# gddickinson/neural_enhanced_super_resolution

Measured on AMD Instinct MI355X. Metric: output megapixels/sec, RealESRGAN_x2plus x2 upscale, higher is better.
Workload: dtype f32 (operands as f16 hi+lo pairs, 3 f16 MFMAs per product, f32 accumulate); 1 GPU; c2: 512x512->1024x1024 RealESRGAN_x2plus fp32 single tile; frames_in_flight_per_gpu=1, world_size=1, partition=independent frames, no data-path collective

## Files before the change

neural_enhanced_super_resolution_amd/csrc/rdb_f16x2.hip:

```cpp
#include <type_traits>

#include "f16x2_common.h"
#include "nesr_kernels.h"
#include "rdb_f16x2_schedule.h"

namespace nesr {

namespace {

#if defined(NESR_RDB_PAR) || defined(NESR_RDB_EPI_STEPS) || defined(NESR_RDB_DMAPRIO) || defined(NESR_RDB_YPRIO) || NESR_RDB_LAG == 0
#error "NESR_RDB_PAR, NESR_RDB_EPI_STEPS, NESR_RDB_DMAPRIO, NESR_RDB_YPRIO and NESR_RDB_LAG=0 were removed; the last commit that had them is 19ed2fc (tools/build_variant.sh 19ed2fc out.so -D... still builds it)"
#endif

#ifndef NESR_RDB_ABL
#define NESR_RDB_ABL 0
#endif
namespace abl {
constexpr bool no_poll = NESR_RDB_ABL & 1;
constexpr bool plain_loads = NESR_RDB_ABL & 2;
constexpr bool plain_stores = NESR_RDB_ABL & 4;
constexpr bool no_mfma = NESR_RDB_ABL & 8;
constexpr bool no_epilogue = NESR_RDB_ABL & 16;
constexpr bool no_in_dma = NESR_RDB_ABL & 32;
constexpr bool no_w_dma = NESR_RDB_ABL & 64;
constexpr bool no_barrier = NESR_RDB_ABL & 512;
constexpr bool no_dma = no_in_dma || no_w_dma;
}

#if NESR_RDB_ABL & 256
__device__ unsigned long long g_rdb_stamps[2][64][8];
__device__ unsigned long long g_rdb_taps[2][8][8];
__device__ unsigned long long g_rdb_arrive[12][8][2];
#define RARRIVE(w, step, ev) do { if (blockIdx.x == 77 && lane == 0 && (step) >= 20 && (step) < 28) { unsigned long long t_ = __builtin_amdgcn_s_memtime(); asm volatile("s_waitcnt lgkmcnt(0)" ::: "memory"); g_rdb_arrive[w][(step) - 20][ev] = t_; } } while (0)
#define RSTAMP(role, step, ev) do { if (blockIdx.x == 77 && lane == 0) { unsigned long long t_ = __builtin_amdgcn_s_memtime(); asm volatile("s_waitcnt lgkmcnt(0)" ::: "memory"); g_rdb_stamps[role][step][ev] = t_; } } while (0)
#define RMSTEP_INIT() int mstep = 0
#define RSTAMP_M(ev) do { if (wave == 1) RSTAMP(0, mstep, ev); } while (0)
#define RARRIVE_M(d, ev) RARRIVE(wave, mstep + (d), ev)
#define RMSTEP_NEXT() ++mstep
#define RKEEP(x, y) asm volatile("" :: "v"(x), "v"(y))
#define RTAPS_INIT() unsigned long long tt_[6]
#define RTAP(i, fence) do { tt_[i] = __builtin_amdgcn_s_memtime(); if (fence) __builtin_amdgcn_sched_barrier(0); } while (0)
#define RTAPS_WRITE() do { if (blockIdx.x == 77 && (wave == 1 || wave == 5) && lane == 0 && mstep >= 20 && mstep < 28) { \
    _Pragma("unroll") for (int i_ = 0; i_ < 6; ++i_) g_rdb_taps[wave == 5][mstep - 20][i_] = tt_[i_]; } } while (0)
#define RCLOCKS(step) do { if (((step) == 0 || (step) == RDB_STEPS - 1) && wave == 0 && blockIdx.x == 77 && lane == 0) { \
    const unsigned long long r_ = __builtin_amdgcn_s_memrealtime(), t_ = __builtin_amdgcn_s_memtime(); asm volatile("s_waitcnt lgkmcnt(0)" ::: "memory"); \
    g_rdb_stamps[1][(step) == 0 ? 62 : 63][0] = r_; g_rdb_stamps[1][(step) == 0 ? 62 : 63][1] = t_; } } while (0)
#define RSTAMP_RETIRED() do { asm volatile("s_waitcnt vmcnt(0)" ::: "memory"); if (wave == 1) RSTAMP(0, 61, 1); } while (0)
#else
#define RSTAMP(role, step, ev) do { } while (0)
#define RARRIVE(w, step, ev) do { } while (0)
#define RMSTEP_INIT() do { } while (0)
#define RSTAMP_M(ev) do { } while (0)
#define RARRIVE_M(d, ev) do { } while (0)
#define RMSTEP_NEXT() do { } while (0)
#define RKEEP(x, y) do { } while (0)
#define RTAPS_INIT() do { } while (0)
#define RTAP(i, fence) do { } while (0)
#define RTAPS_WRITE() do { } while (0)
#define RCLOCKS(step) do { } while (0)
#define RSTAMP_RETIRED() do { } while (0)
#endif

struct RdbArgs {
    const void* cur;
    long long chunk_bytes;
    void* out;
    const void* res2;
    float s1, s2;
    const void* w[5];
    const float* bias[5];
    int n, h, w_;
    unsigned* progress;
    unsigned epoch;
    unsigned* abort_flag;
    unsigned* status;
    unsigned long long timeout_ticks;
};

__device__ __forceinline__ void glds16_s_sc1(const char* sbase, unsigned voff, unsigned lds_dst) {
    unsigned keep;
    asm volatile(
        "s_mov_b32 %0, m0\n\t"
        "s_mov_b32 m0, %3\n\t"
        "s_nop 0\n\t"
        "global_load_lds_dwordx4 %1, %2 sc1\n\t"
        "s_mov_b32 m0, %0"
        : "=&s"(keep)
        : "v"(voff), "s"(sbase), "s"(lds_dst)
        : "memory");
}
__device__ __forceinline__ void store16_wt_s(const char* sbase, unsigned voff, uint4 v) {
    asm volatile("global_store_dwordx4 %0, %1, %2 sc1\n\ts_nop 1" ::"v"(voff), "v"(__builtin_bit_cast(f32x4, v)), "s"(sbase) : "memory");
}
__device__ __forceinline__ f32x4 load16_s(const char* sbase, unsigned voff) {
    return *(const __attribute__((address_space(1))) f32x4*)(sbase + voff);
}

__device__ __forceinline__ void wait_vmcnt_le(int k) {
    switch (k) {
        case 0: asm volatile("s_waitcnt vmcnt(0)" ::: "memory"); break;
        case 1: asm volatile("s_waitcnt vmcnt(1)" ::: "memory"); break;
        case 2: asm volatile("s_waitcnt vmcnt(2)" ::: "memory"); break;
        case 3: asm volatile("s_waitcnt vmcnt(3)" ::: "memory"); break;
        case 4: asm volatile("s_waitcnt vmcnt(4)" ::: "memory"); break;
        case 5: asm volatile("s_waitcnt vmcnt(5)" ::: "memory"); break;
        case 6: asm volatile("s_waitcnt vmcnt(6)" ::: "memory"); break;
        case 7: asm volatile("s_waitcnt vmcnt(7)" ::: "memory"); break;
        case 8: asm volatile("s_waitcnt vmcnt(8)" ::: "memory"); break;
        case 9: asm volatile("s_waitcnt vmcnt(9)" ::: "memory"); break;
        case 10: asm volatile("s_waitcnt vmcnt(10)" ::: "memory"); break;
        case 11: asm volatile("s_waitcnt vmcnt(11)" ::: "memory"); break;
        default: asm volatile("s_waitcnt vmcnt(12)" ::: "memory"); break;
    }
}

constexpr int RSLOTS = 4;
constexpr int W5_ROUNDS = 2 * W_ITEMS / (64 * 4);
static_assert(RSLOTS == 4 && RDB_STEP5 % RSLOTS == 0 && W5_ROUNDS * 64 * 4 == 2 * W_ITEMS, "conv5's slab pairs sit at ring positions 0,1 / 2,3 and fill whole DMA rounds");
constexpr int MW = 8;
constexpr int DW = 4;
constexpr int EPI_STEPS = 1;

__global__ __launch_bounds__(64 * (MW + DW), 3) void rdb_f16x2_kernel(RdbArgs a) {
    typedef Geo<4> G;
    constexpr int THREADS = G::THREADS, TH = G::TH;
    constexpr int IN_ITEMS = G::IN_ITEMS, IN_ROUNDS = G::IN_ROUNDS, IN_BYTES = G::IN_BYTES;
    constexpr int W_ROUNDS = (W_ITEMS + THREADS - 1) / THREADS;
    constexpr int WRING = RSLOTS * IN_BYTES;
    constexpr int BIAS = RSLOTS * (IN_BYTES + W_BYTES);
    static_assert(TH == MW, "one tile row per MFMA wave");
    extern __shared__ __attribute__((aligned(16))) char smem[];

    const int lane = threadIdx.x & 63;
    const int wave_all = __builtin_amdgcn_readfirstlane(threadIdx.x >> 6);
    const bool is_dma = wave_all >= MW;
    const bool is_cmp = !is_dma;
    const int wave = is_cmp ? wave_all : wave_all - MW;
    const int tid = wave * 64 + lane;

    const int tiles_x = (a.w_ + TW - 1) / TW;
    const int tiles_y = (a.h + TH - 1) / TH;
    const int total = tiles_x * tiles_y * a.n;
    const int tile = xcd_work_index(total);
    const int n = tile / (tiles_x * tiles_y);
    const int t2 = tile - n * tiles_x * tiles_y;
    const int ty = t2 / tiles_x, tx = t2 - ty * tiles_x;
    const int y0 = ty * TH, x0 = tx * TW;

    const int j16 = lane & 15, g4 = lane >> 4;
    auto advance = [](int& l, int& c) {
        const int nc = l == 4 ? 12 : 4 + 2 * l;
        if (++c == nc) { c = 0; ++l; }
    };

    if (is_dma) {
        if (wave == 0) RSTAMP(1, 61, 0);
        const unsigned lds_base = (unsigned)(size_t)(lds_char*)(smem);
        unsigned voff[IN_ROUNDS];
        unsigned okmask = 0;
        unsigned wavemask = 0;
        const int row0 = y0 > 0 ? y0 - 1 : 0;
        const char* in_img = static_cast<const char*>(a.cur) + ((size_t)n * a.h + row0) * a.w_ * 64;
        const unsigned* watch = nullptr;
        int kin = 0, kw = 0;
        if (lane < 9) {
            const int ny = ty + lane / 3 - 1, nx = tx + lane % 3 - 1;
            if (ny >= 0 && ny < tiles_y && nx >= 0 && nx < tiles_x) watch = a.progress + (n * tiles_y + ny) * tiles_x + nx;
        }
        {
            int p = tid >> 2;
            int py = p / PW, px = p - py * PW;
            const int sl = tid & 3;
#pragma unroll
            for (int i = 0; i < IN_ROUNDS; ++i) {
                const int k = tid + THREADS * i;
                const int sg = sl ^ (((px >> 2) & 1) << 1);
                const int Y = y0 - 1 + py, X = x0 - 1 + px;
                const bool has = k < IN_ITEMS;
                const bool ok = has && Y >= 0 && Y < a.h && X >= 0 && X < a.w_;
                voff[i] = ((unsigned)(Y - row0) * (unsigned)a.w_ + (unsigned)X) * 64u + sg * 16;
                okmask |= ok ? (1u << i) : 0u;
                if (__builtin_amdgcn_ballot_w64(ok) != 0ull) { wavemask |= 1u << i; ++kin; }
                if (has && !ok) {
#pragma unroll
                    for (int sl2 = 0; sl2 < RSLOTS; ++sl2) *reinterpret_cast<f32x4*>(smem + sl2 * IN_BYTES + k * 16) = f32x4{0.f, 0.f, 0.f, 0.f};
                }
                px += (THREADS / 4) % PW;
                py += (THREADS / 4) / PW;
                if (px >= PW) { px -= PW; py += 1; }
            }
#pragma unroll
            for (int j = 0; j < W_ROUNDS; ++j) kw += (wave * 64 + THREADS * j) < W_ITEMS ? 1 : 0;
        }
        unsigned seen = 0;
        bool gave_up = false;
        auto dma_w = [&](int l, int c, int wpos) {
            const char* wsrc = static_cast<const char*>(a.w[l]) + (size_t)c * W_BYTES;
#pragma unroll
            for (int j = 0; j < W_ROUNDS; ++j) {
                const int k = tid + THREADS * j;
                const unsigned dst = lds_base + WRING + wpos * W_BYTES + j * (THREADS * 16) + wave * 1024;
                if (k < W_ITEMS && !abl::no_w_dma) glds16_s(wsrc, (unsigned)k * 16u, __builtin_amdgcn_readfirstlane(dst));
            }
        };
        auto dma_w5 = [&](int c, int wpos) {
            const char* wsrc = static_cast<const char*>(a.w[4]) + (size_t)c * (2 * W_BYTES);
#pragma unroll
            for (int j = 0; j < W5_ROUNDS; ++j) {
                const unsigned dst = lds_base + WRING + wpos * W_BYTES + j * (THREADS * 16) + wave * 1024;
                if (!abl::no_w_dma) glds16_s(wsrc, (unsigned)(tid + THREADS * j) * 16u, __builtin_amdgcn_readfirstlane(dst));
            }
        };
        auto dma_in = [&](int c, int slot) {
            const unsigned need = c < 4 ? 0u : (unsigned)((c - 4) >> 1) + 1u;
            if (need > seen && !gave_up && !abl::no_poll) {
                const unsigned target = a.epoch + need;
                unsigned long long t0 = 0;
                for (unsigned it = 0;; ++it) {
                    const unsigned v = watch ? __hip_atomic_load(watch, __ATOMIC_RELAXED, __HIP_MEMORY_SCOPE_AGENT) : target;
                    if (__builtin_amdgcn_ballot_w64((int)(v - target) < 0) == 0ull) break;
                    if ((it & 63u) == 0u) {
                        const unsigned long long now = __builtin_amdgcn_s_memrealtime();
                        if (it == 0) t0 = now;
                        const unsigned ab = __hip_atomic_load(a.abort_flag, __ATOMIC_RELAXED, __HIP_MEMORY_SCOPE_AGENT);
                        if (ab != 0u || now - t0 > a.timeout_ticks) {
                            if (ab == 0u && lane == 0) __hip_atomic_store(a.abort_flag, 1u | ((unsigned)c << 8) | ((unsigned)tile << 16), __ATOMIC_RELAXED, __HIP_MEMORY_SCOPE_AGENT);
                            gave_up = true;
                            break;
                        }
                    }
                    __builtin_amdgcn_s_sleep(4);
                }
                seen = need;
            }
            const char* isrc = in_img + (long long)c * a.chunk_bytes;
#pragma unroll
            for (int i = 0; i < IN_ROUNDS; ++i) {
                const unsigned dst = lds_base + slot * IN_BYTES + i * (THREADS * 16) + wave * 1024;
                if (((wavemask >> i) & 1u) && !abl::no_in_dma) {
                    if ((okmask >> i) & 1u) {
                        if (abl::plain_loads) glds16_s(isrc, voff[i], __builtin_amdgcn_readfirstlane(dst));
                        else glds16_s_sc1(isrc, voff[i], __builtin_amdgcn_readfirstlane(dst));
                    }
                }
            }
        };
        int fl = 0, fc = 0;
#pragma unroll
        for (int i = 0; i < rdbs::IN_LEAD; ++i) {
            dma_w(0, i, i);
            dma_in(i, i);
            advance(fl, fc);
        }
        gave_up = *(const __attribute__((address_space(4))) unsigned*)a.abort_flag != 0u;
        asm volatile("s_waitcnt lgkmcnt(0)" ::: "memory");
        int fill = rdbs::IN_LEAD;
        int cl = 0, cc = 0;
        wait_vmcnt_le(abl::no_dma ? 0 : (rdbs::IN_LEAD - 1) * (kw + kin));
        int inflight = kw + kin;
        __builtin_amdgcn_s_barrier();
        asm volatile("" ::: "memory");
        for (int step = 0; step < RDB_STEPS; ++step) {
            if (wave == 0) RSTAMP(1, step, 0);
            RCLOCKS(step);
            wait_vmcnt_le(abl::no_dma ? 0 : inflight);
            if (wave == 0) RSTAMP(1, step, 1);
            RARRIVE(MW + wave, step, 0);
            if (!abl::no_barrier) __builtin_amdgcn_s_barrier();
            asm volatile("" ::: "memory");
            RARRIVE(MW + wave, step, 1);
            if (wave == 0) RSTAMP(1, step, 2);
            if (cc == EPI_STEPS && cl >= 1 && wave == 0 && lane == 0)
                __hip_atomic_store(a.progress + tile, a.epoch + (unsigned)cl, __ATOMIC_RELAXED, __HIP_MEMORY_SCOPE_AGENT);
            if (rdbs::w_pair(step)) {
                dma_w5(step + 1 - RDB_STEP5, ((step + 1) & 1) * 2);
            } else if (rdbs::w_slab(step)) {
                dma_w(fl, fc, fill);
            }
            for (int k = rdbs::in_end(step) - rdbs::in_end(step - 1); k > 0; --k) {
                dma_in(fc, fill);
                advance(fl, fc);
                fill = fill == RSLOTS - 1 ? 0 : fill + 1;
            }
            inflight = rdbs::tail_w(step) * kw + rdbs::tail_in(step) * kin;
            if (wave == 0) RSTAMP(1, step, 3);
            advance(cl, cc);
        }
        return;
    }

    const bool active = (y0 + wave) < a.h;
    if (wave == 1) RSTAMP(0, 61, 0);
    const bool fills_bias = wave < 6 && lane < 8;
    f32x4 bias_v = f32x4{0.f, 0.f, 0.f, 0.f};
    if (fills_bias) bias_v = *(const __attribute__((address_space(1))) f32x4*)(a.bias[wave < 4 ? wave : 4] + (wave == 5 ? 32 : 0) + 4 * lane);
    const int un = g4 >> 1, kh = g4 & 1;
    int b16[5][2], a16[5];
#pragma unroll
    for (int st_ = 0; st_ < 5; ++st_) {
#pragma unroll
        for (int nh = 0; nh < 2; ++nh) b16[st_][nh] = tap_pixel_offset(st_, wave, nh, j16, un, kh);
        a16[st_] = tap_weight_offset(st_, j16, un, kh);
    }
    int slot = 0;
    int wpos = 0;
    RMSTEP_INIT();
    typedef const __attribute__((address_space(3))) f32x4* lds_f32x4;
    const unsigned lds0 = (unsigned)(size_t)(lds_char*)(smem);
    unsigned bcur[5], aw012, aw3, aw4, aw4b;
#pragma unroll
    for (int t = 0; t < 5; ++t) bcur[t] = lds0 + (unsigned)b16[t][0];
    const unsigned xl4 = (unsigned)((un ^ 1) << 5);
    aw012 = lds0 + (unsigned)(WRING + a16[0]);
    aw3 = lds0 + (unsigned)(WRING + a16[3]);
    aw4 = lds0 + (unsigned)(WRING + a16[4]);
    aw4b = aw4 + (unsigned)un * 1024u;
    const int cbl = (g4 & 1) * 16 + (g4 >> 1) * 8;
    const int piece8 = ((g4 & 1) * 2 + (g4 >> 1)) * 8;
    const bool res2 = a.res2 != nullptr;
    f32x4 ep[2][2];
#pragma unroll
    for (int nh = 0; nh < 2; ++nh)
#pragma unroll
        for (int mt = 0; mt < 2; ++mt) ep[nh][mt] = f32x4{0.f, 0.f, 0.f, 0.f};
    int ep_l = -1;
    bool bad = false;
    auto unpack_res = [&](f32x4 rx, f32x4 rx1, f32x4& q0, f32x4& q1) {
        uint4 cx = __builtin_bit_cast(uint4, rx), cx1 = __builtin_bit_cast(uint4, rx1);
        regroup_pairs(cx, cx1);
        const f16x8 h = __builtin_bit_cast(f16x8, cx), lo = __builtin_bit_cast(f16x8, cx1);
#pragma unroll
        for (int i = 0; i < 4; ++i) {
            q0[i] = fmaf((float)lo[i], LO_INV, (float)h[i]);
            q1[i] = fmaf((float)lo[4 + i], LO_INV, (float)h[4 + i]);
        }
    };
    const long long row_bytes = (((long long)n * a.h + (y0 + wave)) * a.w_) * 64;
    unsigned lane_off[2];
    bool lane_ok[2];
#pragma unroll
    for (int nh = 0; nh < 2; ++nh) {
        const int X = x0 + 16 * nh + j16;
        lane_ok[nh] = X < a.w_;
        lane_off[nh] = (unsigned)(lane_ok[nh] ? X : 0) * 64u + (unsigned)piece8 * 2u;
    }
    auto uni = [](const char* p) -> const char* {
        const unsigned long long v = (unsigned long long)p;
        const unsigned lo = __builtin_amdgcn_readfirstlane((unsigned)v), hi = __builtin_amdgcn_readfirstlane((unsigned)(v >> 32));
        return (const char*)(((unsigned long long)hi << 32) | lo);
    };
    auto epi_half = [&](int l, const f32x4& e0, const f32x4& e1, int nh) {
        RSTAMP_M(3);
        const bool valid = lane_ok[nh];
        const unsigned voff = lane_off[nh];
        const char* bsrc = smem + BIAS + (l * 32 + cbl) * 4;
        f32x4 v0, v1;
        cout_exchange(e0, e1, v0, v1);
        v0 += *reinterpret_cast<const f32x4*>(bsrc);
        v1 += *reinterpret_cast<const f32x4*>(bsrc + 16);
        const int dchunk = 4 + 2 * l;
#pragma unroll
        for (int i = 0; i < 4; ++i) { v0[i] = fmaxf(v0[i], v0[i] * 0.2f); v1[i] = fmaxf(v1[i], v1[i] * 0.2f); }
        RKEEP(v0, v1);
        RSTAMP_M(4);
        uint4 cx, cx1;
        bool bad_here = false;
        split_regroup(v0, v1, cx, cx1, bad_here);
        bad |= bad_here && valid;
        RKEEP(__builtin_bit_cast(f32x4, cx), __builtin_bit_cast(f32x4, cx1));
        RSTAMP_M(5);
        if (valid) {
            const char* d0 = uni(static_cast<const char*>(a.cur) + (long long)dchunk * a.chunk_bytes + row_bytes);
            if (!abl::plain_stores) {
                store16_wt_s(d0, voff, cx);
                store16_wt_s(d0 + a.chunk_bytes, voff, cx1);
            } else {
                *reinterpret_cast<uint4*>(const_cast<char*>(d0) + voff) = cx;
                *reinterpret_cast<uint4*>(const_cast<char*>(d0) + a.chunk_bytes + voff) = cx1;
            }
        }
        RSTAMP_M(6);
    };
    auto epi_pending = [&]() {
        if (abl::no_epilogue) return;
        epi_half(ep_l, ep[0][0], ep[0][1], 0);
        epi_half(ep_l, ep[1][0], ep[1][1], 1);
    };
    f32x4 R1[4][2], R2[4][2];
    auto issue_res = [&](const void* base, int g, f32x4 (&R)[4][2]) {
        const char* r = uni(static_cast<const char*>(base) + (long long)(2 * g) * a.chunk_bytes + row_bytes);
#pragma unroll
        for (int nh = 0; nh < 2; ++nh) {
            R[2 * g + nh][0] = load16_s(r, lane_off[nh]);
            R[2 * g + nh][1] = load16_s(r + a.chunk_bytes, lane_off[nh]);
        }
    };
    f32x4 acc16[2][2][2][2];
    f32x4 Af[2][2][2];
    f32x4 Bf[2][2][2];
    auto load_a = [&](int s_, int buf, unsigned off) {
#pragma unroll
        for (int mt = 0; mt < 2; ++mt) {
            if (s_ < 4) {
                const unsigned ad = s_ < 3 ? aw012 + s_ * 2048 : aw3;
                Af[buf][mt][0] = *((lds_f32x4)(size_t)(ad + off + mt * 256));
                Af[buf][mt][1] = *((lds_f32x4)(size_t)(ad + off + mt * 256 + 1024));
            } else {
                f32x4 hi = *((lds_f32x4)(size_t)(aw4 + off + mt * 256));
                Af[buf][mt][1] = *((lds_f32x4)(size_t)(aw4b + off + mt * 256));
                if (un) hi = f32x4{0.f, 0.f, 0.f, 0.f};
                Af[buf][mt][0] = hi;
            }
        }
    };
    auto move_a = [&](unsigned d) {
        aw012 += d;
        aw3 += d;
        aw4 += d;
        aw4b += d;
    };
    auto load_b = [&](int sl, int s_, int buf) {
        const unsigned dB = sl == RSLOTS - 1 ? (unsigned)(-(RSLOTS - 1) * IN_BYTES) : (unsigned)IN_BYTES;
        const unsigned xl = bcur[s_] ^ (s_ == 4 ? xl4 : 32u);
#pragma unroll
        for (int nh = 0; nh < 2; ++nh) {
            Bf[buf][nh][0] = *((lds_f32x4)(size_t)(bcur[s_] + nh * 1024));
            Bf[buf][nh][1] = *((lds_f32x4)(size_t)(xl + nh * 1024));
        }
        bcur[s_] += dB;
    };
    auto mfma_tap = [&](int s_, int g, int abuf, int bbuf) {
#pragma unroll
        for (int mt = 0; mt < 2; ++mt) {
            const f16x8 a0 = __builtin_bit_cast(f16x8, Af[abuf][mt][0]), a1 = __builtin_bit_cast(f16x8, Af[abuf][mt][1]);
#pragma unroll
            for (int nh = 0; nh < 2; ++nh) {
                const f16x8 x0_ = __builtin_bit_cast(f16x8, Bf[bbuf][nh][0]), x1_ = __builtin_bit_cast(f16x8, Bf[bbuf][nh][1]);
                if (s_ < 4) mfma_tap3(a0, a1, x0_, x1_, acc16[g][nh][mt][0], acc16[g][nh][mt][1]);
                else mfma_tap2(a0, a1, x0_, x1_, acc16[g][nh][mt][0], acc16[g][nh][mt][1]);
            }
        }
    };
    auto zero_acc = [&](int g) {
#pragma unroll
        for (int nh = 0; nh < 2; ++nh)
#pragma unroll
            for (int mt = 0; mt < 2; ++mt)
#pragma unroll
                for (int q = 0; q < 2; ++q) acc16[g][nh][mt][q] = f32x4{0.f, 0.f, 0.f, 0.f};
    };
    auto step_body = [&](auto Pc, auto Mc, int c) {
        constexpr int P = decltype(Pc)::value, M = decltype(Mc)::value;
        constexpr int BT = rdbs::bar_tap(M);
        auto bar = [&](int cb) {
            if (cb == EPI_STEPS) asm volatile("s_waitcnt vmcnt(0)" ::: "memory");
            RSTAMP_M(0);
            RARRIVE_M(cb - c, 0);
            if (!abl::no_barrier) __builtin_amdgcn_s_barrier();
            asm volatile("" ::: "memory");
            RARRIVE_M(cb - c, 1);
            RSTAMP_M(1);
        };
        if (rdbs::bar_top(M)) bar(c);
        const bool epi_now = active && ep_l >= 0 && c < EPI_STEPS;
        const int nslot = slot == RSLOTS - 1 ? 0 : slot + 1;
        const unsigned dA = wpos == RSLOTS - 1 ? (unsigned)(-(RSLOTS - 1) * W_BYTES) : (unsigned)W_BYTES;
        if (!active || abl::no_mfma) {
            if (BT >= 0) bar(c + 1);
        } else {
            if (rdbs::req_behind(M)) {
                load_a(0, P, 0);
                load_b(slot, 0, P);
            }
            if (epi_now) {
                epi_pending();
                __builtin_amdgcn_sched_barrier(0);
            }
            RTAPS_INIT();
#pragma unroll
            for (int s_ = 0; s_ < 5; ++s_) {
                const int buf = (s_ + P) & 1;
                RTAP(s_, true);
                if (s_ == BT) {
                    bar(c + 1);
                    __builtin_amdgcn_sched_barrier(0);
                }
                if (s_ + 1 < 5) {
                    load_a(s_ + 1, buf ^ 1, 0);
                    load_b(slot, s_ + 1, buf ^ 1);
                } else if (rdbs::req_early(M)) {
                    load_a(0, buf ^ 1, dA);
                    load_b(nslot, 0, buf ^ 1);
                }
                mfma_tap(s_, 0, buf, buf);
                if (s_ + 1 < 5 || rdbs::req_early(M)) {
#pragma unroll
                    for (int i = 0; i < 8; ++i) {
                        __builtin_amdgcn_sched_group_barrier(0x008, 1, 0);
                        __builtin_amdgcn_sched_group_barrier(0x100, 1, 0);
                    }
                }
                __builtin_amdgcn_sched_barrier(0);
            }
            RTAP(5, false);
            RTAPS_WRITE();
        }
        move_a(dA);
        slot = nslot;
        wpos = wpos == RSLOTS - 1 ? 0 : wpos + 1;
        RSTAMP_M(2);
        RMSTEP_NEXT();
    };
    auto step_body5 = [&](auto Pc, auto Fc, auto Lc, int c) {
        constexpr int P = decltype(Pc)::value;
        constexpr bool FIRST = decltype(Fc)::value == 1;
        constexpr bool last_of_all = decltype(Lc)::value != 0;
        if (c == EPI_STEPS) asm volatile("s_waitcnt vmcnt(0)" ::: "memory");
        RSTAMP_M(0);
        RARRIVE_M(0, 0);
        if (!abl::no_barrier) __builtin_amdgcn_s_barrier();
        asm volatile("" ::: "memory");
        RARRIVE_M(0, 1);
        RSTAMP_M(1);
        const bool epi_now = active && ep_l >= 0 && c < EPI_STEPS;
        const int nslot = slot == RSLOTS - 1 ? 0 : slot + 1;
        const unsigned dA = wpos == 0 ? (unsigned)(2 * W_BYTES) : (unsigned)(-2 * W_BYTES);
        if (active && !abl::no_mfma) {
            load_a(0, 0, 0);
            if (FIRST) load_b(slot, 0, P);
            if (epi_now) {
                epi_pending();
                __builtin_amdgcn_sched_barrier(0);
            }
            if (FIRST) { zero_acc(0); zero_acc(1); }
#pragma unroll
            for (int s_ = 0; s_ < 5; ++s_) {
                const int buf = (s_ + P) & 1;
                if (last_of_all && s_ == 4 && !abl::no_epilogue) {
                    issue_res(a.cur, 0, R1);
                    asm volatile("" ::: "memory");
                    __builtin_amdgcn_sched_barrier(0);
                }
                load_a(s_, 1, W_BYTES);
                if (s_ + 1 < 5) load_b(slot, s_ + 1, buf ^ 1);
                else if (!last_of_all) load_b(nslot, 0, buf ^ 1);
                mfma_tap(s_, 0, 0, buf);
#pragma unroll
                for (int i = 0; i < 8; ++i) {
                    __builtin_amdgcn_sched_group_barrier(0x008, 1, 0);
                    __builtin_amdgcn_sched_group_barrier(0x100, 1, 0);
                }
                __builtin_amdgcn_sched_barrier(0);
                if (s_ + 1 < 5) load_a(s_ + 1, 0, 0);
                else if (last_of_all && !abl::no_epilogue) {
                    issue_res(a.cur, 1, R1);
                    asm volatile("" ::: "memory");
                    __builtin_amdgcn_sched_barrier(0);
                }
                mfma_tap(s_, 1, 1, buf);
                if (s_ + 1 < 5) {
#pragma unroll
                    for (int i = 0; i < 4; ++i) {
                        __builtin_amdgcn_sched_group_barrier(0x008, 2, 0);
                        __builtin_amdgcn_sched_group_barrier(0x100, 1, 0);
                    }
                }
                __builtin_amdgcn_sched_barrier(0);
            }
        }
        move_a(dA);
        slot = nslot;
        wpos = wpos == 0 ? 2 : 0;
        RSTAMP_M(2);
        RMSTEP_NEXT();
    };
    if (fills_bias) *reinterpret_cast<f32x4*>(smem + BIAS + wave * 128 + lane * 16) = bias_v;
    asm volatile("s_waitcnt lgkmcnt(0)" ::: "memory");
    __builtin_amdgcn_s_barrier();
    asm volatile("" ::: "memory");
    typedef std::integral_constant<int, 0> I0;
    typedef std::integral_constant<int, 1> I1;
    typedef std::integral_constant<int, rdbs::M_LEAD> MLead;
    typedef std::integral_constant<int, rdbs::M_LAG_FIRST> MFirst;
    typedef std::integral_constant<int, rdbs::M_LAG_MID> MMid;
    typedef std::integral_constant<int, rdbs::M_LAG_LAST> MLast;
    static_assert(rdbs::mode_of(true, 4) == rdbs::M_LAG_FIRST && rdbs::mode_of(true, 5) == rdbs::M_LAG_MID &&
                  rdbs::mode_of(true, 8) == rdbs::M_LAG_MID && rdbs::mode_of(true, 9) == rdbs::M_LAG_LAST &&
                  rdbs::mode_of(false, 0) == rdbs::M_LEAD && rdbs::mode_of(false, RDB_STEP5 - 1) == rdbs::M_LEAD, "the loops below are the walk's sequence");
    auto layer_done = [&](int l) {
#pragma unroll
        for (int nh = 0; nh < 2; ++nh)
#pragma unroll
            for (int mt = 0; mt < 2; ++mt)
#pragma unroll
                for (int i = 0; i < 4; ++i) ep[nh][mt][i] = fmaf(acc16[0][nh][mt][1][i], LO_INV, acc16[0][nh][mt][0][i]);
        ep_l = l;
    };
    if (wave < 4) {
        for (int l = 0; l < 4; ++l) {
            const int nc = 4 + 2 * l;
            zero_acc(0);
            for (int c = 0; c < nc; c += 2) {
                step_body(I0{}, MLead{}, c);
                step_body(I1{}, MLead{}, c + 1);
            }
            layer_done(l);
        }
    } else {
        for (int l = 0; l < 4; ++l) {
            const int nc = 4 + 2 * l;
            zero_acc(0);
            step_body(I0{}, MFirst{}, 0);
            for (int c = 1; c < nc - 1; c += 2) {
                step_body(I1{}, MMid{}, c);
                step_body(I0{}, MMid{}, c + 1);
            }
            step_body(I1{}, MLast{}, nc - 1);
            layer_done(l);
        }
    }
    step_body5(I0{}, I1{}, I0{}, 0);
    step_body5(I1{}, I0{}, I0{}, 1);
    for (int c = 2; c < 10; c += 2) {
        step_body5(I0{}, I0{}, I0{}, c);
        step_body5(I1{}, I0{}, I0{}, c + 1);
    }
    step_body5(I0{}, I0{}, I0{}, 10);
    step_body5(I1{}, I0{}, I1{}, 11);
    auto final_epilogue = [&](auto Rc) {
        constexpr bool RES2 = decltype(Rc)::value != 0;
        if (RES2) {
            issue_res(a.res2, 0, R2);
            issue_res(a.res2, 1, R2);
        }
        asm volatile("" ::: "memory");
        __builtin_amdgcn_sched_barrier(0);
        RSTAMP_M(3);
        uint4 cx[4], cx1[4];
#pragma unroll
        for (int p = 0; p < 4; ++p) {
            const int g = p >> 1, nh = p & 1;
            f32x4 e0, e1;
#pragma unroll
            for (int i = 0; i < 4; ++i) {
                e0[i] = fmaf(acc16[g][nh][0][1][i], LO_INV, acc16[g][nh][0][0][i]);
                e1[i] = fmaf(acc16[g][nh][1][1][i], LO_INV, acc16[g][nh][1][0][i]);
            }
            const char* bsrc = smem + BIAS + (4 * 32 + 32 * g + cbl) * 4;
            f32x4 v0, v1;
            cout_exchange(e0, e1, v0, v1);
            v0 += *reinterpret_cast<const f32x4*>(bsrc);
            v1 += *reinterpret_cast<const f32x4*>(bsrc + 16);
            f32x4 q0, q1;
            unpack_res(R1[p][0], R1[p][1], q0, q1);
#pragma unroll
            for (int i = 0; i < 4; ++i) { v0[i] = __fadd_rn(__fmul_rn(v0[i], a.s1), q0[i]); v1[i] = __fadd_rn(__fmul_rn(v1[i], a.s1), q1[i]); }
            if (RES2) {
                unpack_res(R2[p][0], R2[p][1], q0, q1);
#pragma unroll
                for (int i = 0; i < 4; ++i) { v0[i] = __fadd_rn(__fmul_rn(v0[i], a.s2), q0[i]); v1[i] = __fadd_rn(__fmul_rn(v1[i], a.s2), q1[i]); }
            }
            bool bad_here = false;
            split_regroup(v0, v1, cx[p], cx1[p], bad_here);
            bad |= bad_here && lane_ok[nh];
            __builtin_amdgcn_sched_barrier(0);
        }
        RSTAMP_M(5);
#pragma unroll
        for (int p = 0; p < 4; ++p) {
            if (lane_ok[p & 1]) {
                const char* d0 = uni(static_cast<const char*>(a.out) + (long long)(2 * (p >> 1)) * a.chunk_bytes + row_bytes);
                store16_wt_s(d0, lane_off[p & 1], cx[p]);
                store16_wt_s(d0 + a.chunk_bytes, lane_off[p & 1], cx1[p]);
            }
        }
        RSTAMP_M(6);
        RSTAMP_RETIRED();
    };
    if (active && !abl::no_epilogue) {
        if (res2) final_epilogue(I1{});
        else final_epilogue(I0{});
    }
    if (bad && a.status) __hip_atomic_store(a.status, 1u, __ATOMIC_RELAXED, __HIP_MEMORY_SCOPE_AGENT);
}

}

#if NESR_RDB_ABL & 256
extern "C" int nesr_debug_rdb_steps() { return RDB_STEPS; }
extern "C" int nesr_debug_rdb_stamps(unsigned long long* out) {
    return (int)hipMemcpyFromSymbol(out, HIP_SYMBOL(g_rdb_stamps), sizeof(unsigned long long) * 2 * 64 * 8);
}
extern "C" int nesr_debug_rdb_taps(unsigned long long* out) {
    return (int)hipMemcpyFromSymbol(out, HIP_SYMBOL(g_rdb_taps), sizeof(unsigned long long) * 2 * 8 * 8);
}
extern "C" int nesr_debug_rdb_arrive(unsigned long long* out) {
    return (int)hipMemcpyFromSymbol(out, HIP_SYMBOL(g_rdb_arrive), sizeof(unsigned long long) * 12 * 8 * 2);
}
#endif

int rdb_f16x2_tiles(int n, int h, int w) { return ((w + TW - 1) / TW) * ((h + 7) / 8) * n; }

hipError_t launch_rdb_f16x2(const RdbLaunch& r, hipStream_t s) {
    typedef Geo<4> G;
    constexpr size_t shm = (size_t)RSLOTS * (G::IN_BYTES + (size_t)W_BYTES) + 768;
    static unsigned long long attr_done = 0;
    {
        const hipError_t e = ensure_dynamic_lds(reinterpret_cast<const void*>(&rdb_f16x2_kernel), shm, attr_done);
        if (e != hipSuccess) return e;
    }
    if ((long long)r.w_ * 64 * 12 >= (1ll << 32)) return hipErrorInvalidValue;
    RdbArgs a;
    a.cur = r.cur; a.chunk_bytes = r.chunk_bytes; a.out = r.out; a.res2 = r.res2; a.s1 = r.s1; a.s2 = r.s2;
    for (int i = 0; i < 5; ++i) { a.w[i] = r.w[i]; a.bias[i] = r.bias[i]; }
    a.n = r.n; a.h = r.h; a.w_ = r.w_;
    a.progress = r.progress; a.epoch = r.epoch; a.abort_flag = r.abort_flag; a.status = r.status;
    a.timeout_ticks = r.timeout_ticks ? r.timeout_ticks : 20000000ull;
    int total = rdb_f16x2_tiles(r.n, r.h, r.w_);
    if (total <= 0) return hipSuccess;
    static int resident = -1;
    if (resident < 0) {
        int per_cu = 0, dev = 0, cus = 0;
        if (hipOccupancyMaxActiveBlocksPerMultiprocessor(&per_cu, rdb_f16x2_kernel, 64 * (MW + DW), shm) != hipSuccess || hipGetDevice(&dev) != hipSuccess ||
            hipDeviceGetAttribute(&cus, hipDeviceAttributeMultiprocessorCount, dev) != hipSuccess)
            return hipErrorUnknown;
        resident = per_cu * cus;
    }
    if (total > resident) return hipErrorLaunchOutOfResources;
    total -= r.debug_drop;
    if (total <= 0) return hipSuccess;
    hipLaunchKernelGGL(rdb_f16x2_kernel, dim3((unsigned)total), dim3(64 * (MW + DW)), shm, s, a);
    return hipGetLastError();
}

}
```

neural_enhanced_super_resolution_amd/csrc/rdb_f16x2_schedule.h:

```cpp
#pragma once

namespace nesr {

constexpr int RDB_STEP5 = 4 + 6 + 8 + 10;
constexpr int RDB_STEPS = RDB_STEP5 + 12;

#ifndef NESR_RDB_LAG
#define NESR_RDB_LAG 2
#endif
namespace rdbs {
constexpr int LAG = NESR_RDB_LAG;
static_assert(LAG == 2 || LAG == 3, "NESR_RDB_LAG: 2 (barrier in front of tap-step 3) or 3 (in front of tap-step 2)");
constexpr int layer_of(int s) { return s < 4 ? 0 : s < 10 ? 1 : s < 18 ? 2 : s < RDB_STEP5 ? 3 : 4; }
constexpr int first_of(int l) { return l == 0 ? 0 : l == 1 ? 4 : l == 2 ? 10 : l == 3 ? 18 : RDB_STEP5; }
constexpr int steps_of(int l) { return l == 4 ? RDB_STEPS - RDB_STEP5 : 4 + 2 * l; }
enum Mode {
    M_LEAD,
    M_LAG_FIRST,
    M_LAG_MID,
    M_LAG_LAST,
    M_CONV5
};
constexpr int mode_of(bool lagging, int s) {
    const int l = layer_of(s), c = s - first_of(l);
    return l == 4 ? M_CONV5 : !lagging ? M_LEAD : c == 0 ? M_LAG_FIRST : c == steps_of(l) - 1 ? M_LAG_LAST : M_LAG_MID;
}
constexpr bool bar_top(int m) { return m != M_LAG_MID && m != M_LAG_LAST; }
constexpr int bar_tap(int m) { return m == M_LAG_FIRST || m == M_LAG_MID ? 5 - LAG : -1; }
constexpr bool req_behind(int m) { return m == M_LEAD || m == M_LAG_FIRST; }
constexpr bool req_early(int m) { return m == M_LAG_FIRST || m == M_LAG_MID; }
constexpr int in_end(int i) {
    const int e = i < RDB_STEP5 ? i + 3 : i + 4;
    return e < RDB_STEPS ? e : RDB_STEPS;
}
constexpr int IN_LEAD = in_end(-1);
constexpr bool w_slab(int i) { return i + 1 < RDB_STEP5 && in_end(i - 1) < RDB_STEP5; }
constexpr bool w_pair(int i) { return i + 1 >= RDB_STEP5 && i + 1 < RDB_STEPS; }
constexpr int tail_w(int i) { return w_slab(i) ? 1 : 0;}
constexpr int tail_in(int i) {
    const int n = in_end(i) - in_end(i - 1);
    return i == RDB_STEP5 - 1 ? 0
         : i == RDB_STEP5 ? 1
         : n;
}
struct Walk {
    int in_iss[RDB_STEPS] = {}, w_iss[RDB_STEPS] = {};
    int in_land[RDB_STEPS] = {}, w_land[RDB_STEPS] = {};
    int rd_lo[2][RDB_STEPS + 1] = {}, rd_hi[2][RDB_STEPS + 1] = {};
    int wr_hi[2][RDB_STEPS + 1] = {};
    int bars[3] = {};
    bool ok = true;
};
constexpr bool pos_overlap_w(int t, int u) {
    const int t0 = t < RDB_STEP5 ? (t & 3) : (t & 1) * 2, t1 = t < RDB_STEP5 ? t0 : t0 + 1;
    const int u0 = u < RDB_STEP5 ? (u & 3) : (u & 1) * 2, u1 = u < RDB_STEP5 ? u0 : u0 + 1;
    return t0 <= u1 && u0 <= t1;
}
constexpr Walk walk() {
    Walk k;
    for (int r = 0; r < 2; ++r) {
        for (int i = 0; i <= RDB_STEPS; ++i) { k.rd_lo[r][i] = RDB_STEPS; k.rd_hi[r][i] = -1; k.wr_hi[r][i] = -1; }
        int b = 1;
        auto rd = [&](int t, bool pix, bool wts) {
            if (t < k.rd_lo[r][b - 1]) k.rd_lo[r][b - 1] = t;
            if (pix && t > k.rd_hi[r][b - 1]) k.rd_hi[r][b - 1] = t;
            if (wts && t > k.wr_hi[r][b - 1]) k.wr_hi[r][b - 1] = t;
        };
        for (int s = 0; s < RDB_STEPS; ++s) {
            const int m = mode_of(r, s);
            if (bar_top(m)) ++b;
            for (int t = 0; t < 5; ++t) {
                if (t == bar_tap(m)) ++b;
                rd(s, true, true);
                if (t == 4 && req_early(m)) rd(s + 1, true, s + 1 < RDB_STEP5);
                if (t == 4 && m == M_CONV5 && s + 1 < RDB_STEPS) rd(s + 1, true, false);
            }
        }
        k.bars[r] = b;
    }
    int q_step[3 * RDB_STEPS] = {}, q_w[3 * RDB_STEPS] = {}, qn = 0, landed = 0;
    auto land = [&](int upto, int b) {
        for (; landed < upto; ++landed) (q_w[landed] ? k.w_land : k.in_land)[q_step[landed]] = b;
    };
    for (int t = 0; t < IN_LEAD; ++t) {
        q_step[qn] = t; q_w[qn++] = 1; k.w_iss[t] = -2;
        q_step[qn] = t; q_w[qn++] = 0; k.in_iss[t] = -2;
    }
    land(qn - 2 * (IN_LEAD - 1), -1);
    int tail = 2;
    k.bars[2] = 1;
    for (int i = 0; i < RDB_STEPS; ++i) {
        land(qn - tail, i);
        ++k.bars[2];
        const int f = in_end(i - 1), e = in_end(i);
        if (w_pair(i)) { q_step[qn] = i + 1; q_w[qn++] = 1; k.w_iss[i + 1] = i; }
        else if (w_slab(i)) {
            if (e - f != 1) k.ok = false;
            q_step[qn] = f; q_w[qn++] = 1; k.w_iss[f] = i;
        }
        for (int t = f; t < e; ++t) { q_step[qn] = t; q_w[qn++] = 0; k.in_iss[t] = i; }
        tail = tail_w(i) + tail_in(i);
        if (tail_w(i) && tail_in(i) != e - f) k.ok = false;
    }
    if (qn != 2 * RDB_STEPS) k.ok = false;
    land(qn, RDB_STEPS);
    for (int r = 0; r < 2; ++r)
        for (int i = -1; i < RDB_STEPS; ++i) {
            for (int t = k.rd_lo[r][i + 1]; t <= k.rd_hi[r][i + 1]; ++t) {
                if (k.in_land[t] > i) k.ok = false;
                for (int u = t + 1; u < RDB_STEPS; ++u) if ((u & 3) == (t & 3) && k.in_iss[u] <= i) k.ok = false;
            }
            for (int t = k.rd_lo[r][i + 1]; t <= k.wr_hi[r][i + 1]; ++t) {
                if (k.w_land[t] > i) k.ok = false;
                for (int u = t + 1; u < RDB_STEPS; ++u) if (pos_overlap_w(t, u) && k.w_iss[u] <= i) k.ok = false;
            }
        }
    return k;
}
constexpr Walk WALK = walk();
static_assert(WALK.ok, "a ring position is refilled while it is read, or read before the wait that covers it");
static_assert(WALK.bars[0] == RDB_STEPS + 1 && WALK.bars[1] == RDB_STEPS + 1 && WALK.bars[2] == RDB_STEPS + 1, "every role takes the same number of barriers");
}

}
```

Baseline: 173.3 MP/s.

## Drive RDB DMA and compute steps from a compile-time step table

Replaces the hard-coded layer/chunk advance logic with a constexpr step table that encodes, per step, which weight slabs and input chunks to prefetch, the ring positions to use and the wait depths. The DMA waves read packed words from constant memory, and the lookahead is now computed by a planner, so weights can be issued further ahead (vmcnt waits up to 24). The compute side gains per-step accumulator zeroing, lane-epilogue values recomputed on demand to lower register pressure, and masking in place of branches. The cost is more complex scheduling plus constant-memory reads, and a risk of different register allocation or deeper in-flight DMA contending with other traffic.

Result: slower. 171.3 MP/s (-1.2%).

```diff
diff --git a/neural_enhanced_super_resolution_amd/csrc/rdb_f16x2.hip b/neural_enhanced_super_resolution_amd/csrc/rdb_f16x2.hip
--- a/neural_enhanced_super_resolution_amd/csrc/rdb_f16x2.hip
+++ b/neural_enhanced_super_resolution_amd/csrc/rdb_f16x2.hip
@@ -110,16 +110,29 @@
         case 9: asm volatile("s_waitcnt vmcnt(9)" ::: "memory"); break;
         case 10: asm volatile("s_waitcnt vmcnt(10)" ::: "memory"); break;
         case 11: asm volatile("s_waitcnt vmcnt(11)" ::: "memory"); break;
-        default: asm volatile("s_waitcnt vmcnt(12)" ::: "memory"); break;
+        case 12: asm volatile("s_waitcnt vmcnt(12)" ::: "memory"); break;
+        case 13: asm volatile("s_waitcnt vmcnt(13)" ::: "memory"); break;
+        case 14: asm volatile("s_waitcnt vmcnt(14)" ::: "memory"); break;
+        case 15: asm volatile("s_waitcnt vmcnt(15)" ::: "memory"); break;
+        case 16: asm volatile("s_waitcnt vmcnt(16)" ::: "memory"); break;
+        case 17: asm volatile("s_waitcnt vmcnt(17)" ::: "memory"); break;
+        case 18: asm volatile("s_waitcnt vmcnt(18)" ::: "memory"); break;
+        case 19: asm volatile("s_waitcnt vmcnt(19)" ::: "memory"); break;
+        case 20: asm volatile("s_waitcnt vmcnt(20)" ::: "memory"); break;
+        case 21: asm volatile("s_waitcnt vmcnt(21)" ::: "memory"); break;
+        case 22: asm volatile("s_waitcnt vmcnt(22)" ::: "memory"); break;
+        case 23: asm volatile("s_waitcnt vmcnt(23)" ::: "memory"); break;
+        default: asm volatile("s_waitcnt vmcnt(24)" ::: "memory"); break;
     }
 }
 
 constexpr int RSLOTS = 4;
-constexpr int W5_ROUNDS = 2 * W_ITEMS / (64 * 4);
-static_assert(RSLOTS == 4 && RDB_STEP5 % RSLOTS == 0 && W5_ROUNDS * 64 * 4 == 2 * W_ITEMS, "conv5's slab pairs sit at ring positions 0,1 / 2,3 and fill whole DMA rounds");
+static_assert(RSLOTS == 4, "the step table puts a D-step's slab pair at ring positions 0,1 / 2,3");
 constexpr int MW = 8;
 constexpr int DW = 4;
 constexpr int EPI_STEPS = 1;
+
+__constant__ rdbs::Words SCHED = rdbs::WORDS;
 
 __global__ __launch_bounds__(64 * (MW + DW), 3) void rdb_f16x2_kernel(RdbArgs a) {
     typedef Geo<4> G;
@@ -148,11 +161,6 @@
     const int y0 = ty * TH, x0 = tx * TW;
 
     const int j16 = lane & 15, g4 = lane >> 4;
-    auto advance = [](int& l, int& c) {
-        const int nc = l == 4 ? 12 : 4 + 2 * l;
-        if (++c == nc) { c = 0; ++l; }
-    };
-
     if (is_dma) {
         if (wave == 0) RSTAMP(1, 61, 0);
         const unsigned lds_base = (unsigned)(size_t)(lds_char*)(smem);
@@ -194,8 +202,8 @@
         }
         unsigned seen = 0;
         bool gave_up = false;
-        auto dma_w = [&](int l, int c, int wpos) {
-            const char* wsrc = static_cast<const char*>(a.w[l]) + (size_t)c * W_BYTES;
+        auto dma_w = [&](int l, int idx, int wpos) {
+            const char* wsrc = static_cast<const char*>(a.w[l]) + (size_t)idx * W_BYTES;
 #pragma unroll
             for (int j = 0; j < W_ROUNDS; ++j) {
                 const int k = tid + THREADS * j;
@@ -203,12 +211,14 @@
                 if (k < W_ITEMS && !abl::no_w_dma) glds16_s(wsrc, (unsigned)k * 16u, __builtin_amdgcn_readfirstlane(dst));
             }
         };
-        auto dma_w5 = [&](int c, int wpos) {
-            const char* wsrc = static_cast<const char*>(a.w[4]) + (size_t)c * (2 * W_BYTES);
-#pragma unroll
-            for (int j = 0; j < W5_ROUNDS; ++j) {
-                const unsigned dst = lds_base + WRING + wpos * W_BYTES + j * (THREADS * 16) + wave * 1024;
-                if (!abl::no_w_dma) glds16_s(wsrc, (unsigned)(tid + THREADS * j) * 16u, __builtin_amdgcn_readfirstlane(dst));
+        auto dma_w_step = [&](unsigned sw) {
+            const int wp = (int)(sw >> 21) & 3;
+            const int la = (int)((sw >> 5) & 7u) - 1, ia = (int)(sw >> 8) & 31, lb = (int)((sw >> 13) & 7u) - 1, ib = (int)(sw >> 16) & 31;
+            if (sw & 16u) {
+                dma_w(la, ia, wp);
+                dma_w(lb, ib, wp + 1);
+            } else {
+                dma_w(la >= 0 ? la : lb, la >= 0 ? ia : ib, wp);
             }
         };
         auto dma_in = [&](int c, int slot) {
@@ -245,22 +255,23 @@
                 }
             }
         };
-        int fl = 0, fc = 0;
-#pragma unroll
-        for (int i = 0; i < rdbs::IN_LEAD; ++i) {
-            dma_w(0, i, i);
-            dma_in(i, i);
-            advance(fl, fc);
-        }
+#pragma unroll
+        for (int t = 0; t < rdbs::PRO_W; ++t) dma_w_step(rdbs::step_word(t));
+#pragma unroll
+        for (int t = 0; t < rdbs::PRO_IN; ++t) dma_in(rdbs::TAB.s[t].chunk, t & (RSLOTS - 1));
+#pragma unroll
+        for (int t = rdbs::PRO_W; t < rdbs::W_LEAD; ++t) dma_w_step(rdbs::step_word(t));
+#pragma unroll
+        for (int t = rdbs::PRO_IN; t < rdbs::IN_LEAD; ++t) dma_in(rdbs::TAB.s[t].chunk, t & (RSLOTS - 1));
         gave_up = *(const __attribute__((address_space(4))) unsigned*)a.abort_flag != 0u;
         asm volatile("s_waitcnt lgkmcnt(0)" ::: "memory");
-        int fill = rdbs::IN_LEAD;
-        int cl = 0, cc = 0;
-        wait_vmcnt_le(abl::no_dma ? 0 : (rdbs::IN_LEAD - 1) * (kw + kin));
-        int inflight = kw + kin;
+        int fw = rdbs::W_LEAD, fi = rdbs::IN_LEAD;
+        int inflight = rdbs::tail_w(-1) * kw + rdbs::tail_in(-1) * kin;
+        wait_vmcnt_le(abl::no_dma ? 0 : inflight);
         __builtin_amdgcn_s_barrier();
         asm volatile("" ::: "memory");
         for (int step = 0; step < RDB_STEPS; ++step) {
+            const unsigned iw = SCHED.iv[step];
             if (wave == 0) RSTAMP(1, step, 0);
             RCLOCKS(step);
             wait_vmcnt_le(abl::no_dma ? 0 : inflight);
@@ -270,21 +281,16 @@
             asm volatile("" ::: "memory");
             RARRIVE(MW + wave, step, 1);
             if (wave == 0) RSTAMP(1, step, 2);
-            if (cc == EPI_STEPS && cl >= 1 && wave == 0 && lane == 0)
-                __hip_atomic_store(a.progress + tile, a.epoch + (unsigned)cl, __ATOMIC_RELAXED, __HIP_MEMORY_SCOPE_AGENT);
-            if (rdbs::w_pair(step)) {
-                dma_w5(step + 1 - RDB_STEP5, ((step + 1) & 1) * 2);
-            } else if (rdbs::w_slab(step)) {
-                dma_w(fl, fc, fill);
-            }
-            for (int k = rdbs::in_end(step) - rdbs::in_end(step - 1); k > 0; --k) {
-                dma_in(fc, fill);
-                advance(fl, fc);
-                fill = fill == RSLOTS - 1 ? 0 : fill + 1;
-            }
-            inflight = rdbs::tail_w(step) * kw + rdbs::tail_in(step) * kin;
+            const unsigned pub = (iw >> 9) & 7u;
+            if (pub != 0u && wave == 0 && lane == 0)
+                __hip_atomic_store(a.progress + tile, a.epoch + pub, __ATOMIC_RELAXED, __HIP_MEMORY_SCOPE_AGENT);
+            for (int k = (int)(iw & 3u); k > 0; --k) dma_w_step(SCHED.st[fw++]);
+            for (int k = (int)((iw >> 2) & 3u); k > 0; --k) {
+                dma_in((int)(SCHED.st[fi] & 15u), fi & (RSLOTS - 1));
+                ++fi;
+            }
+            inflight = (int)((iw >> 4) & 7u) * kw + (int)((iw >> 7) & 3u) * kin;
             if (wave == 0) RSTAMP(1, step, 3);
-            advance(cl, cc);
         }
         return;
     }
@@ -308,15 +314,24 @@
     typedef const __attribute__((address_space(3))) f32x4* lds_f32x4;
     const unsigned lds0 = (unsigned)(size_t)(lds_char*)(smem);
     unsigned bcur[5], aw012, aw3, aw4, aw4b;
+#if NESR_RDB_ABL & 256
+#define RING_OPAQUE() do { slot = __builtin_amdgcn_readfirstlane(slot); wpos = __builtin_amdgcn_readfirstlane(wpos); asm volatile("" : "+s"(slot), "+s"(wpos)); } while (0)
+#else
+#define RING_OPAQUE() asm volatile("" : "+s"(slot), "+s"(wpos))
+#endif
 #pragma unroll
     for (int t = 0; t < 5; ++t) bcur[t] = lds0 + (unsigned)b16[t][0];
-    const unsigned xl4 = (unsigned)((un ^ 1) << 5);
+    unsigned unm = un ? 0u : 0xffffffffu;
+    asm volatile("" : "+v"(unm));
     aw012 = lds0 + (unsigned)(WRING + a16[0]);
     aw3 = lds0 + (unsigned)(WRING + a16[3]);
     aw4 = lds0 + (unsigned)(WRING + a16[4]);
     aw4b = aw4 + (unsigned)un * 1024u;
-    const int cbl = (g4 & 1) * 16 + (g4 >> 1) * 8;
-    const int piece8 = ((g4 & 1) * 2 + (g4 >> 1)) * 8;
+    struct LaneEp {
+        int cbl;
+        unsigned off[2];
+        bool ok[2];
+    };
     const bool res2 = a.res2 != nullptr;
     f32x4 ep[2][2];
 #pragma unroll
@@ -336,24 +351,31 @@
         }
     };
     const long long row_bytes = (((long long)n * a.h + (y0 + wave)) * a.w_) * 64;
-    unsigned lane_off[2];
-    bool lane_ok[2];
-#pragma unroll
-    for (int nh = 0; nh < 2; ++nh) {
-        const int X = x0 + 16 * nh + j16;
-        lane_ok[nh] = X < a.w_;
-        lane_off[nh] = (unsigned)(lane_ok[nh] ? X : 0) * 64u + (unsigned)piece8 * 2u;
-    }
+    auto lane_ep = [&]() __attribute__((always_inline)) {
+        LaneEp e;
+        unsigned ln;
+        asm volatile("v_mbcnt_lo_u32_b32 %0, -1, 0\n\tv_mbcnt_hi_u32_b32 %0, -1, %0" : "=v"(ln));
+        const int j = (int)(ln & 15u), g = (int)(ln >> 4);
+        e.cbl = (g & 1) * 16 + (g >> 1) * 8;
+        const int piece8 = ((g & 1) * 2 + (g >> 1)) * 8;
+#pragma unroll
+        for (int nh = 0; nh < 2; ++nh) {
+            const int X = x0 + 16 * nh + j;
+            e.ok[nh] = X < a.w_;
+            e.off[nh] = (unsigned)(e.ok[nh] ? X : 0) * 64u + (unsigned)piece8 * 2u;
+        }
+        return e;
+    };
     auto uni = [](const char* p) -> const char* {
         const unsigned long long v = (unsigned long long)p;
         const unsigned lo = __builtin_amdgcn_readfirstlane((unsigned)v), hi = __builtin_amdgcn_readfirstlane((unsigned)(v >> 32));
         return (const char*)(((unsigned long long)hi << 32) | lo);
     };
-    auto epi_half = [&](int l, const f32x4& e0, const f32x4& e1, int nh) {
+    auto epi_half = [&](const LaneEp& le, int l, const f32x4& e0, const f32x4& e1, int nh) {
         RSTAMP_M(3);
-        const bool valid = lane_ok[nh];
-        const unsigned voff = lane_off[nh];
-        const char* bsrc = smem + BIAS + (l * 32 + cbl) * 4;
+        const bool valid = le.ok[nh];
+        const unsigned voff = le.off[nh];
+        const char* bsrc = smem + BIAS + (l * 32 + le.cbl) * 4;
         f32x4 v0, v1;
         cout_exchange(e0, e1, v0, v1);
         v0 += *reinterpret_cast<const f32x4*>(bsrc);
@@ -383,16 +405,19 @@
     };
     auto epi_pending = [&]() {
         if (abl::no_epilogue) return;
-        epi_half(ep_l, ep[0][0], ep[0][1], 0);
-        epi_half(ep_l, ep[1][0], ep[1][1], 1);
+        int l = ep_l;
+        asm volatile("" : "+s"(l));
+        const LaneEp le = lane_ep();
+        epi_half(le, l, ep[0][0], ep[0][1], 0);
+        epi_half(le, l, ep[1][0], ep[1][1], 1);
     };
     f32x4 R1[4][2], R2[4][2];
-    auto issue_res = [&](const void* base, int g, f32x4 (&R)[4][2]) {
+    auto issue_res = [&](const LaneEp& le, const void* base, int g, f32x4 (&R)[4][2]) {
         const char* r = uni(static_cast<const char*>(base) + (long long)(2 * g) * a.chunk_bytes + row_bytes);
 #pragma unroll
         for (int nh = 0; nh < 2; ++nh) {
-            R[2 * g + nh][0] = load16_s(r, lane_off[nh]);
-            R[2 * g + nh][1] = load16_s(r + a.chunk_bytes, lane_off[nh]);
+            R[2 * g + nh][0] = load16_s(r, le.off[nh]);
+            R[2 * g + nh][1] = load16_s(r + a.chunk_bytes, le.off[nh]);
         }
     };
     f32x4 acc16[2][2][2][2];
@@ -408,8 +433,9 @@
             } else {
                 f32x4 hi = *((lds_f32x4)(size_t)(aw4 + off + mt * 256));
                 Af[buf][mt][1] = *((lds_f32x4)(size_t)(aw4b + off + mt * 256));
-                if (un) hi = f32x4{0.f, 0.f, 0.f, 0.f};
-                Af[buf][mt][0] = hi;
+                uint4 hb = __builtin_bit_cast(uint4, hi);
+                hb.x &= unm; hb.y &= unm; hb.z &= unm; hb.w &= unm;
+                Af[buf][mt][0] = __builtin_bit_cast(f32x4, hb);
             }
         }
     };
@@ -418,16 +444,18 @@
         aw3 += d;
         aw4 += d;
         aw4b += d;
+        asm volatile("" : "+v"(aw012), "+v"(aw3), "+v"(aw4), "+v"(aw4b));
     };
     auto load_b = [&](int sl, int s_, int buf) {
         const unsigned dB = sl == RSLOTS - 1 ? (unsigned)(-(RSLOTS - 1) * IN_BYTES) : (unsigned)IN_BYTES;
-        const unsigned xl = bcur[s_] ^ (s_ == 4 ? xl4 : 32u);
+        const unsigned xl = bcur[s_] ^ (s_ == 4 ? (unm & 32u) : 32u);
 #pragma unroll
         for (int nh = 0; nh < 2; ++nh) {
             Bf[buf][nh][0] = *((lds_f32x4)(size_t)(bcur[s_] + nh * 1024));
             Bf[buf][nh][1] = *((lds_f32x4)(size_t)(xl + nh * 1024));
         }
         bcur[s_] += dB;
+        asm volatile("" : "+v"(bcur[s_]));
     };
     auto mfma_tap = [&](int s_, int g, int abuf, int bbuf) {
 #pragma unroll
@@ -449,8 +477,8 @@
 #pragma unroll
                 for (int q = 0; q < 2; ++q) acc16[g][nh][mt][q] = f32x4{0.f, 0.f, 0.f, 0.f};
     };
-    auto step_body = [&](auto Pc, auto Mc, int c) {
-        constexpr int P = decltype(Pc)::value, M = decltype(Mc)::value;
+    auto step_body = [&](auto Pc, auto Mc, auto Gc, int c, bool zero) __attribute__((always_inline)) {
+        constexpr int P = decltype(Pc)::value, M = decltype(Mc)::value, G = decltype(Gc)::value;
         constexpr int BT = rdbs::bar_tap(M);
         auto bar = [&](int cb) {
             if (cb == EPI_STEPS) asm volatile("s_waitcnt vmcnt(0)" ::: "memory");
@@ -476,6 +504,7 @@
                 epi_pending();
                 __builtin_amdgcn_sched_barrier(0);
             }
+            if (zero) zero_acc(G);
             RTAPS_INIT();
 #pragma unroll
             for (int s_ = 0; s_ < 5; ++s_) {
@@ -492,7 +521,7 @@
                     load_a(0, buf ^ 1, dA);
                     load_b(nslot, 0, buf ^ 1);
                 }
-                mfma_tap(s_, 0, buf, buf);
+                mfma_tap(s_, G, buf, buf);
                 if (s_ + 1 < 5 || rdbs::req_early(M)) {
 #pragma unroll
                     for (int i = 0; i < 8; ++i) {
@@ -508,13 +537,14 @@
         move_a(dA);
         slot = nslot;
         wpos = wpos == RSLOTS - 1 ? 0 : wpos + 1;
+        RING_OPAQUE();
         RSTAMP_M(2);
         RMSTEP_NEXT();
     };
-    auto step_body5 = [&](auto Pc, auto Fc, auto Lc, int c) {
+    auto step_body5 = [&](auto Pc, auto Fc, auto Lc, int c, int zero, bool last_of_all) __attribute__((always_inline)) {
         constexpr int P = decltype(Pc)::value;
         constexpr bool FIRST = decltype(Fc)::value == 1;
-        constexpr bool last_of_all = decltype(Lc)::value != 0;
+        constexpr bool LAST = decltype(Lc)::value != 0;
         if (c == EPI_STEPS) asm volatile("s_waitcnt vmcnt(0)" ::: "memory");
         RSTAMP_M(0);
         RARRIVE_M(0, 0);
@@ -532,18 +562,22 @@
                 epi_pending();
                 __builtin_amdgcn_sched_barrier(0);
             }
-            if (FIRST) { zero_acc(0); zero_acc(1); }
+            if (FIRST) {
+                if (zero & 1) zero_acc(0);
+                if (zero & 2) zero_acc(1);
+                __builtin_amdgcn_sched_barrier(0);
+            }
 #pragma unroll
             for (int s_ = 0; s_ < 5; ++s_) {
                 const int buf = (s_ + P) & 1;
-                if (last_of_all && s_ == 4 && !abl::no_epilogue) {
-                    issue_res(a.cur, 0, R1);
+                if (LAST && last_of_all && s_ == 4 && !abl::no_epilogue) {
+                    issue_res(lane_ep(), a.cur, 0, R1);
                     asm volatile("" ::: "memory");
                     __builtin_amdgcn_sched_barrier(0);
                 }
                 load_a(s_, 1, W_BYTES);
                 if (s_ + 1 < 5) load_b(slot, s_ + 1, buf ^ 1);
-                else if (!last_of_all) load_b(nslot, 0, buf ^ 1);
+                else if (!LAST) load_b(nslot, 0, buf ^ 1);
                 mfma_tap(s_, 0, 0, buf);
 #pragma unroll
                 for (int i = 0; i < 8; ++i) {
@@ -552,8 +586,8 @@
                 }
                 __builtin_amdgcn_sched_barrier(0);
                 if (s_ + 1 < 5) load_a(s_ + 1, 0, 0);
-                else if (last_of_all && !abl::no_epilogue) {
-                    issue_res(a.cur, 1, R1);
+                else if (LAST && last_of_all && !abl::no_epilogue) {
+                    issue_res(lane_ep(), a.cur, 1, R1);
                     asm volatile("" ::: "memory");
                     __builtin_amdgcn_sched_barrier(0);
                 }
@@ -571,6 +605,7 @@
         move_a(dA);
         slot = nslot;
         wpos = wpos == 0 ? 2 : 0;
+        RING_OPAQUE();
         RSTAMP_M(2);
         RMSTEP_NEXT();
     };
@@ -584,55 +619,96 @@
     typedef std::integral_constant<int, rdbs::M_LAG_FIRST> MFirst;
     typedef std::integral_constant<int, rdbs::M_LAG_MID> MMid;
     typedef std::integral_constant<int, rdbs::M_LAG_LAST> MLast;
-    static_assert(rdbs::mode_of(true, 4) == rdbs::M_LAG_FIRST && rdbs::mode_of(true, 5) == rdbs::M_LAG_MID &&
-                  rdbs::mode_of(true, 8) == rdbs::M_LAG_MID && rdbs::mode_of(true, 9) == rdbs::M_LAG_LAST &&
-                  rdbs::mode_of(false, 0) == rdbs::M_LEAD && rdbs::mode_of(false, RDB_STEP5 - 1) == rdbs::M_LEAD, "the loops below are the walk's sequence");
-    auto layer_done = [&](int l) {
+    auto layer_done = [&](auto Gc, int l) __attribute__((always_inline)) {
+        constexpr int G = decltype(Gc)::value;
 #pragma unroll
         for (int nh = 0; nh < 2; ++nh)
 #pragma unroll
             for (int mt = 0; mt < 2; ++mt)
 #pragma unroll
-                for (int i = 0; i < 4; ++i) ep[nh][mt][i] = fmaf(acc16[0][nh][mt][1][i], LO_INV, acc16[0][nh][mt][0][i]);
+                for (int i = 0; i < 4; ++i) ep[nh][mt][i] = fmaf(acc16[G][nh][mt][1][i], LO_INV, acc16[G][nh][mt][0][i]);
         ep_l = l;
     };
+    auto run_d = [&](auto Nc, auto Hc, int zero, bool last_of_all) __attribute__((always_inline)) {
+        constexpr int N = decltype(Nc)::value;
+        constexpr bool HEAD = decltype(Hc)::value != 0;
+        step_body5(I0{}, I1{}, std::integral_constant<int, HEAD>{}, 0, zero, false);
+        if (N > 2) {
+            step_body5(I1{}, std::integral_constant<int, HEAD>{}, I0{}, 1, 0, false);
+            for (int c = 2; c < N - 2; c += 2) {
+                step_body5(I0{}, I0{}, I0{}, c, 0, false);
+                step_body5(I1{}, I0{}, I0{}, c + 1, 0, false);
+            }
+            step_body5(I0{}, I0{}, I0{}, N - 2, 0, false);
+        }
+        step_body5(I1{}, I0{}, I1{}, N - 1, 0, last_of_all);
+    };
+    auto run_s_lead = [&](auto Gc, int n, bool zero) __attribute__((always_inline)) {
+        step_body(I0{}, MLead{}, Gc, 0, zero);
+        step_body(I1{}, MLead{}, Gc, 1, false);
+        for (int c = 2; c < n; c += 2) {
+            step_body(I0{}, MLead{}, Gc, c, false);
+            step_body(I1{}, MLead{}, Gc, c + 1, false);
+        }
+    };
+    auto run_s_lag = [&](auto Gc, int n, bool zero) __attribute__((always_inline)) {
+        step_body(I0{}, MFirst{}, Gc, 0, zero);
+        for (int c = 1; c < n - 1; c += 2) {
+            step_body(I1{}, MMid{}, Gc, c, false);
+            step_body(I0{}, MMid{}, Gc, c + 1, false);
+        }
+        step_body(I1{}, MLast{}, Gc, n - 1, false);
+    };
+    {
+        using namespace rdbs;
+        constexpr auto is = [](int r, int kind, int n, int la, int lb) {
+            return RUNS[r].kind == kind && RUNS[r].n == n && RUNS[r].la == la && RUNS[r].lb == lb;
+        };
+        static_assert(NRUNS == 7 && is(0, K_D, 4, 0, 1) && is(1, K_S, 4, 2, -1) && is(2, K_D, 2, 2, 1) && is(3, K_S, 4, -1, 3) &&
+                      is(4, K_S, 2, 2, -1) && is(5, K_S, 6, -1, 3) && is(6, K_D, 12, 4, 4), "the loops below are the step table's runs");
+        static_assert(TAB.s[0].zero == 3 && TAB.s[4].zero == 1 && TAB.s[8].zero == 0 && TAB.s[10].zero == 2 && TAB.s[14].zero == 0 &&
+                      TAB.s[16].zero == 0 && TAB.s[RDB_STEP5].zero == 3, "where a set starts at zero");
+        static_assert(TAB.s[3].done == 0 && TAB.s[3].done_set == 0 && TAB.s[9].done == 1 && TAB.s[9].done_set == 1 &&
+                      TAB.s[15].done == 2 && TAB.s[15].done_set == 0 && TAB.s[21].done == 3 && TAB.s[21].done_set == 1, "where a layer is complete, and in which set");
+        static_assert(mode_of(true, 4) == M_LAG_FIRST && mode_of(true, 5) == M_LAG_MID && mode_of(true, 7) == M_LAG_LAST &&
+                      mode_of(true, 14) == M_LAG_FIRST && mode_of(true, 15) == M_LAG_LAST && mode_of(false, 4) == M_LEAD &&
+                      mode_of(true, 8) == M_CONV5 && d_prefetch(8) && !d_prefetch(9) && !d_prefetch(3) && !d_prefetch(0) && d_prefetch(1), "the loops below are the walk's sequence");
+    }
+    typedef std::integral_constant<int, 2> I2;
+    typedef std::integral_constant<int, 4> I4;
+    typedef std::integral_constant<int, 12> I12;
     if (wave < 4) {
-        for (int l = 0; l < 4; ++l) {
-            const int nc = 4 + 2 * l;
-            zero_acc(0);
-            for (int c = 0; c < nc; c += 2) {
-                step_body(I0{}, MLead{}, c);
-                step_body(I1{}, MLead{}, c + 1);
-            }
-            layer_done(l);
-        }
+        run_d(I4{}, I1{}, 3, false);
+        layer_done(I0{}, 0);
+        run_s_lead(I0{}, 4, true);
+        ep_l = -1;
+        run_d(I2{}, I0{}, 0, false);
+        layer_done(I1{}, 1);
+        run_s_lead(I1{}, 4, true);
+        ep_l = -1;
+        run_s_lead(I0{}, 2, false);
+        layer_done(I0{}, 2);
+        run_s_lead(I1{}, 6, false);
+        layer_done(I1{}, 3);
     } else {
-        for (int l = 0; l < 4; ++l) {
-            const int nc = 4 + 2 * l;
-            zero_acc(0);
-            step_body(I0{}, MFirst{}, 0);
-            for (int c = 1; c < nc - 1; c += 2) {
-                step_body(I1{}, MMid{}, c);
-                step_body(I0{}, MMid{}, c + 1);
-            }
-            step_body(I1{}, MLast{}, nc - 1);
-            layer_done(l);
-        }
+        run_d(I4{}, I1{}, 3, false);
+        layer_done(I0{}, 0);
+        run_s_lag(I0{}, 4, true);
+        ep_l = -1;
+        run_d(I2{}, I0{}, 0, false);
+        layer_done(I1{}, 1);
+        run_s_lag(I1{}, 4, true);
+        ep_l = -1;
+        run_s_lag(I0{}, 2, false);
+        layer_done(I0{}, 2);
+        run_s_lag(I1{}, 6, false);
+        layer_done(I1{}, 3);
     }
-    step_body5(I0{}, I1{}, I0{}, 0);
-    step_body5(I1{}, I0{}, I0{}, 1);
-    for (int c = 2; c < 10; c += 2) {
-        step_body5(I0{}, I0{}, I0{}, c);
-        step_body5(I1{}, I0{}, I0{}, c + 1);
-    }
-    step_body5(I0{}, I0{}, I0{}, 10);
-    step_body5(I1{}, I0{}, I1{}, 11);
+    run_d(I12{}, I0{}, 3, true);
     auto final_epilogue = [&](auto Rc) {
         constexpr bool RES2 = decltype(Rc)::value != 0;
-        if (RES2) {
-            issue_res(a.res2, 0, R2);
-            issue_res(a.res2, 1, R2);
-        }
+        const LaneEp le = lane_ep();
+        if (RES2) issue_res(le, a.res2, 0, R2);
         asm volatile("" ::: "memory");
         __builtin_amdgcn_sched_barrier(0);
         RSTAMP_M(3);
@@ -646,7 +722,7 @@
                 e0[i] = fmaf(acc16[g][nh][0][1][i], LO_INV, acc16[g][nh][0][0][i]);
                 e1[i] = fmaf(acc16[g][nh][1][1][i], LO_INV, acc16[g][nh][1][0][i]);
             }
-            const char* bsrc = smem + BIAS + (4 * 32 + 32 * g + cbl) * 4;
+            const char* bsrc = smem + BIAS + (4 * 32 + 32 * g + le.cbl) * 4;
             f32x4 v0, v1;
             cout_exchange(e0, e1, v0, v1);
             v0 += *reinterpret_cast<const f32x4*>(bsrc);
@@ -662,16 +738,21 @@
             }
             bool bad_here = false;
             split_regroup(v0, v1, cx[p], cx1[p], bad_here);
-            bad |= bad_here && lane_ok[nh];
+            bad |= bad_here && le.ok[nh];
             __builtin_amdgcn_sched_barrier(0);
+            if (RES2 && p == 0) {
+                issue_res(le, a.res2, 1, R2);
+                asm volatile("" ::: "memory");
+                __builtin_amdgcn_sched_barrier(0);
+            }
         }
         RSTAMP_M(5);
 #pragma unroll
         for (int p = 0; p < 4; ++p) {
-            if (lane_ok[p & 1]) {
+            if (le.ok[p & 1]) {
                 const char* d0 = uni(static_cast<const char*>(a.out) + (long long)(2 * (p >> 1)) * a.chunk_bytes + row_bytes);
-                store16_wt_s(d0, lane_off[p & 1], cx[p]);
-                store16_wt_s(d0 + a.chunk_bytes, lane_off[p & 1], cx1[p]);
+                store16_wt_s(d0, le.off[p & 1], cx[p]);
+                store16_wt_s(d0 + a.chunk_bytes, le.off[p & 1], cx1[p]);
             }
         }
         RSTAMP_M(6);
diff --git a/neural_enhanced_super_resolution_amd/csrc/rdb_f16x2_schedule.h b/neural_enhanced_super_resolution_amd/csrc/rdb_f16x2_schedule.h
--- a/neural_enhanced_super_resolution_amd/csrc/rdb_f16x2_schedule.h
+++ b/neural_enhanced_super_resolution_amd/csrc/rdb_f16x2_schedule.h
@@ -1,9 +1,6 @@
 #pragma once
 
 namespace nesr {
-
-constexpr int RDB_STEP5 = 4 + 6 + 8 + 10;
-constexpr int RDB_STEPS = RDB_STEP5 + 12;
 
 #ifndef NESR_RDB_LAG
 #define NESR_RDB_LAG 2
@@ -11,9 +8,77 @@
 namespace rdbs {
 constexpr int LAG = NESR_RDB_LAG;
 static_assert(LAG == 2 || LAG == 3, "NESR_RDB_LAG: 2 (barrier in front of tap-step 3) or 3 (in front of tap-step 2)");
-constexpr int layer_of(int s) { return s < 4 ? 0 : s < 10 ? 1 : s < 18 ? 2 : s < RDB_STEP5 ? 3 : 4; }
-constexpr int first_of(int l) { return l == 0 ? 0 : l == 1 ? 4 : l == 2 ? 10 : l == 3 ? 18 : RDB_STEP5; }
-constexpr int steps_of(int l) { return l == 4 ? RDB_STEPS - RDB_STEP5 : 4 + 2 * l; }
+
+enum Kind { K_S = 0, K_D = 1 };
+struct Run {
+    int kind, n, ch0;
+    int la, lb;
+};
+constexpr int NRUNS = 7;
+constexpr Run RUNS[NRUNS] = {
+    {K_D, 4, 0, 0, 1},
+    {K_S, 4, 0, 2, -1},
+    {K_D, 2, 4, 2, 1},
+    {K_S, 4, 0, -1, 3},
+    {K_S, 2, 6, 2, -1},
+    {K_S, 6, 4, -1, 3},
+    {K_D, 12, 0, 4, 4},
+};
+constexpr int count_steps(int upto) { int n = 0; for (int r = 0; r < upto; ++r) n += RUNS[r].n; return n; }
+}
+constexpr int RDB_STEPS = rdbs::count_steps(rdbs::NRUNS);
+constexpr int RDB_STEP5 = rdbs::count_steps(rdbs::NRUNS - 1);
+namespace rdbs {
+constexpr int chunks_of(int l) { return l == 4 ? 12 : 4 + 2 * l; }
+struct Step {
+    int kind, run, c, n;
+    int chunk;
+    int layer[2], widx[2];
+    int wpos;
+    int epi, epi_set;
+    int zero;
+    int done, done_set;
+};
+struct Table { Step s[RDB_STEPS] = {}; bool ok = true; };
+constexpr Table make_table() {
+    Table t;
+    int k = 0, wp = 0, pend = -1, pend_set = -1;
+    for (int r = 0; r < NRUNS; ++r) {
+        const Run& u = RUNS[r];
+        if (u.n < 2 || (u.n & 1)) t.ok = false;
+        for (int c = 0; c < u.n; ++c, ++k) {
+            Step& s = t.s[k];
+            s.kind = u.kind; s.run = r; s.c = c; s.n = u.n; s.chunk = u.ch0 + c;
+            s.zero = 0; s.done = -1; s.done_set = -1;
+            for (int g = 0; g < 2; ++g) {
+                const int l = g ? u.lb : u.la;
+                s.layer[g] = l;
+                s.widx[g] = l < 0 ? 0 : l == 4 ? 2 * s.chunk + g : s.chunk;
+                if (l >= 0 && s.chunk >= chunks_of(l)) t.ok = false;
+                if (l >= 0 && c == 0 && u.ch0 == 0) s.zero |= 1 << g;
+            }
+            if (u.kind == K_D ? (u.la < 0 || u.lb < 0) : ((u.la < 0) == (u.lb < 0))) t.ok = false;
+            if (u.kind == K_D) { if (wp & 1) t.ok = false; s.wpos = wp; wp = (wp + 2) & 3; }
+            else { s.wpos = wp; wp = (wp + 1) & 3; }
+            s.epi = c == 0 ? pend : -1;
+            s.epi_set = c == 0 ? pend_set : -1;
+            if (c == 0) { pend = -1; pend_set = -1; }
+        }
+        for (int g = 0; g < 2; ++g) {
+            const int l = g ? u.lb : u.la;
+            if (l >= 0 && l < 4 && u.ch0 + u.n == chunks_of(l)) {
+                if (pend >= 0) t.ok = false;
+                pend = l; pend_set = g;
+                t.s[k - 1].done = l; t.s[k - 1].done_set = g;
+            }
+        }
+    }
+    return t;
+}
+constexpr Table TAB = make_table();
+static_assert(TAB.ok, "the run list is not a schedule the kernel can run");
+constexpr int publish(int s) { return s >= 1 && TAB.s[s - 1].epi >= 0 ? TAB.s[s - 1].epi + 1 : 0; }
+
 enum Mode {
     M_LEAD,
     M_LAG_FIRST,
@@ -22,103 +87,185 @@
     M_CONV5
 };
 constexpr int mode_of(bool lagging, int s) {
-    const int l = layer_of(s), c = s - first_of(l);
-    return l == 4 ? M_CONV5 : !lagging ? M_LEAD : c == 0 ? M_LAG_FIRST : c == steps_of(l) - 1 ? M_LAG_LAST : M_LAG_MID;
+    const Step& t = TAB.s[s];
+    return t.kind == K_D ? M_CONV5 : !lagging ? M_LEAD : t.c == 0 ? M_LAG_FIRST : t.c == t.n - 1 ? M_LAG_LAST : M_LAG_MID;
 }
 constexpr bool bar_top(int m) { return m != M_LAG_MID && m != M_LAG_LAST; }
 constexpr int bar_tap(int m) { return m == M_LAG_FIRST || m == M_LAG_MID ? 5 - LAG : -1; }
 constexpr bool req_behind(int m) { return m == M_LEAD || m == M_LAG_FIRST; }
 constexpr bool req_early(int m) { return m == M_LAG_FIRST || m == M_LAG_MID; }
-constexpr int in_end(int i) {
-    const int e = i < RDB_STEP5 ? i + 3 : i + 4;
-    return e < RDB_STEPS ? e : RDB_STEPS;
-}
-constexpr int IN_LEAD = in_end(-1);
-constexpr bool w_slab(int i) { return i + 1 < RDB_STEP5 && in_end(i - 1) < RDB_STEP5; }
-constexpr bool w_pair(int i) { return i + 1 >= RDB_STEP5 && i + 1 < RDB_STEPS; }
-constexpr int tail_w(int i) { return w_slab(i) ? 1 : 0;}
-constexpr int tail_in(int i) {
-    const int n = in_end(i) - in_end(i - 1);
-    return i == RDB_STEP5 - 1 ? 0
-         : i == RDB_STEP5 ? 1
-         : n;
-}
-struct Walk {
-    int in_iss[RDB_STEPS] = {}, w_iss[RDB_STEPS] = {};
-    int in_land[RDB_STEPS] = {}, w_land[RDB_STEPS] = {};
-    int rd_lo[2][RDB_STEPS + 1] = {}, rd_hi[2][RDB_STEPS + 1] = {};
-    int wr_hi[2][RDB_STEPS + 1] = {};
-    int bars[3] = {};
-    bool ok = true;
-};
-constexpr bool pos_overlap_w(int t, int u) {
-    const int t0 = t < RDB_STEP5 ? (t & 3) : (t & 1) * 2, t1 = t < RDB_STEP5 ? t0 : t0 + 1;
-    const int u0 = u < RDB_STEP5 ? (u & 3) : (u & 1) * 2, u1 = u < RDB_STEP5 ? u0 : u0 + 1;
-    return t0 <= u1 && u0 <= t1;
-}
-constexpr Walk walk() {
-    Walk k;
+constexpr bool d_prefetch(int s) { return s > 0 && TAB.s[s].kind == K_D && TAB.s[s].c + 1 < TAB.s[s].n; }
+
+constexpr int NI = RDB_STEPS + 1;
+struct Reads {
+    int lo[2][NI] = {}, hi[2][NI] = {}, whi[2][NI] = {};
+    int bars[2] = {};
+};
+constexpr Reads reads() {
+    Reads k;
     for (int r = 0; r < 2; ++r) {
-        for (int i = 0; i <= RDB_STEPS; ++i) { k.rd_lo[r][i] = RDB_STEPS; k.rd_hi[r][i] = -1; k.wr_hi[r][i] = -1; }
+        for (int i = 0; i < NI; ++i) { k.lo[r][i] = RDB_STEPS; k.hi[r][i] = -1; k.whi[r][i] = -1; }
         int b = 1;
-        auto rd = [&](int t, bool pix, bool wts) {
-            if (t < k.rd_lo[r][b - 1]) k.rd_lo[r][b - 1] = t;
-            if (pix && t > k.rd_hi[r][b - 1]) k.rd_hi[r][b - 1] = t;
-            if (wts && t > k.wr_hi[r][b - 1]) k.wr_hi[r][b - 1] = t;
-        };
         for (int s = 0; s < RDB_STEPS; ++s) {
             const int m = mode_of(r, s);
             if (bar_top(m)) ++b;
             for (int t = 0; t < 5; ++t) {
                 if (t == bar_tap(m)) ++b;
-                rd(s, true, true);
-                if (t == 4 && req_early(m)) rd(s + 1, true, s + 1 < RDB_STEP5);
-                if (t == 4 && m == M_CONV5 && s + 1 < RDB_STEPS) rd(s + 1, true, false);
+                const int i = b - 1;
+                if (s < k.lo[r][i]) k.lo[r][i] = s;
+                if (s > k.hi[r][i]) k.hi[r][i] = s;
+                if (s > k.whi[r][i]) k.whi[r][i] = s;
+                if (t == 4 && req_early(m)) { k.hi[r][i] = s + 1; k.whi[r][i] = s + 1; }
+                if (t == 4 && d_prefetch(s)) k.hi[r][i] = s + 1;
             }
         }
         k.bars[r] = b;
     }
-    int q_step[3 * RDB_STEPS] = {}, q_w[3 * RDB_STEPS] = {}, qn = 0, landed = 0;
-    auto land = [&](int upto, int b) {
-        for (; landed < upto; ++landed) (q_w[landed] ? k.w_land : k.in_land)[q_step[landed]] = b;
-    };
-    for (int t = 0; t < IN_LEAD; ++t) {
-        q_step[qn] = t; q_w[qn++] = 1; k.w_iss[t] = -2;
-        q_step[qn] = t; q_w[qn++] = 0; k.in_iss[t] = -2;
-    }
-    land(qn - 2 * (IN_LEAD - 1), -1);
-    int tail = 2;
+    return k;
+}
+constexpr Reads READS = reads();
+constexpr int min2(int a, int b) { return a < b ? a : b; }
+constexpr int max2(int a, int b) { return a > b ? a : b; }
+constexpr int lo_of(int i) { return i < 0 ? 0 : min2(READS.lo[0][i + 1], READS.lo[1][i + 1]); }
+constexpr bool w_overlap(int t, int u) {
+    const int t0 = TAB.s[t].wpos, t1 = t0 + TAB.s[t].kind, u0 = TAB.s[u].wpos, u1 = u0 + TAB.s[u].kind;
+    return t0 <= u1 && u0 <= t1;
+}
+struct Plan {
+    int in_end[NI] = {}, w_end[NI] = {};
+    int tail_w[NI] = {}, tail_in[NI] = {};
+    bool ok = true;
+};
+constexpr int PRO_IN = max2(READS.hi[0][1], READS.hi[1][1]) + 1, PRO_W = max2(READS.whi[0][1], READS.whi[1][1]) + 1;
+struct Queue {
+    int step[2 * RDB_STEPS] = {}, w[2 * RDB_STEPS] = {}, n = 0;
+    constexpr void push(int s, int is_w) { step[n] = s; w[n] = is_w; ++n; }
+};
+constexpr Plan plan() {
+    Plan p;
+    Queue q;
+    int fw = 0, fi = 0;
+    for (int i = -1; i < RDB_STEPS; ++i) {
+        const int lo = lo_of(i);
+        int we = fw, ie = fi;
+        for (; we < RDB_STEPS; ++we) {
+            bool busy = false;
+            for (int t = lo; t < we; ++t) busy = busy || w_overlap(t, we);
+            if (busy) break;
+        }
+        ie = min2(RDB_STEPS, lo + 4);
+        if (ie < fi) p.ok = false;
+        if (i < 0) {
+            if (PRO_W > we || PRO_IN > ie) p.ok = false;
+            for (int t = 0; t < PRO_W; ++t) q.push(t, 1);
+            for (int t = 0; t < PRO_IN; ++t) q.push(t, 0);
+            for (int t = PRO_W; t < we; ++t) q.push(t, 1);
+            for (int t = PRO_IN; t < ie; ++t) q.push(t, 0);
+        } else {
+            for (int t = fw; t < we; ++t) q.push(t, 1);
+            for (int t = fi; t < ie; ++t) q.push(t, 0);
+        }
+        fw = we; fi = ie;
+        p.w_end[i + 1] = we; p.in_end[i + 1] = ie;
+        int last = -1;
+        if (i + 1 < RDB_STEPS) {
+            const int need_in = max2(READS.hi[0][i + 2], READS.hi[1][i + 2]), need_w = max2(READS.whi[0][i + 2], READS.whi[1][i + 2]);
+            for (int j = 0; j < q.n; ++j) if (q.step[j] <= (q.w[j] ? need_w : need_in)) last = j;
+            if (need_in >= ie || need_w >= we) p.ok = false;
+        } else last = q.n - 1;
+        for (int j = last + 1; j < q.n; ++j) { if (q.w[j]) p.tail_w[i + 1] += 1 + TAB.s[q.step[j]].kind; else ++p.tail_in[i + 1]; }
+    }
+    if (fw != RDB_STEPS || fi != RDB_STEPS) p.ok = false;
+    return p;
+}
+constexpr Plan PLAN = plan();
+static_assert(PLAN.ok, "the DMA plan does not cover the step table");
+constexpr int in_end(int i) { return PLAN.in_end[i + 1]; }
+constexpr int w_end(int i) { return PLAN.w_end[i + 1]; }
+constexpr int tail_w(int i) { return PLAN.tail_w[i + 1]; }
+constexpr int tail_in(int i) { return PLAN.tail_in[i + 1]; }
+constexpr int IN_LEAD = in_end(-1), W_LEAD = w_end(-1);
+
+constexpr unsigned interval_word(int i) {
+    return (unsigned)(w_end(i) - w_end(i - 1)) | (unsigned)(in_end(i) - in_end(i - 1)) << 2 | (unsigned)tail_w(i) << 4 |
+           (unsigned)tail_in(i) << 7 | (unsigned)publish(i) << 9;
+}
+constexpr unsigned step_word(int s) {
+    const Step& t = TAB.s[s];
+    return (unsigned)t.chunk | (unsigned)t.kind << 4 | (unsigned)(t.layer[0] + 1) << 5 | (unsigned)t.widx[0] << 8 |
+           (unsigned)(t.layer[1] + 1) << 13 | (unsigned)t.widx[1] << 16 | (unsigned)t.wpos << 21;
+}
+struct Words { unsigned iv[RDB_STEPS] = {}, st[RDB_STEPS] = {}; bool ok = true; };
+constexpr Words words() {
+    Words w;
+    for (int i = 0; i < RDB_STEPS; ++i) {
+        w.iv[i] = interval_word(i);
+        w.st[i] = step_word(i);
+        if (w_end(i) - w_end(i - 1) > 3 || in_end(i) - in_end(i - 1) > 3 || tail_w(i) > 7 || tail_in(i) > 3) w.ok = false;
+    }
+    return w;
+}
+constexpr Words WORDS = words();
+static_assert(WORDS.ok, "a count does not fit its field");
+
+struct Walk {
+    int in_iss[RDB_STEPS] = {}, w_iss[RDB_STEPS] = {};
+    int in_land[RDB_STEPS] = {}, w_land[RDB_STEPS] = {};
+    int bars[3] = {};
+    bool ok = true;
+};
+constexpr Walk walk() {
+    Walk k;
+    k.bars[0] = READS.bars[0]; k.bars[1] = READS.bars[1];
+    Queue q;
+    int landed = 0;
     k.bars[2] = 1;
-    for (int i = 0; i < RDB_STEPS; ++i) {
-        land(qn - tail, i);
+    for (int i = -1; i < RDB_STEPS; ++i) {
+        const int w0 = i < 0 ? 0 : w_end(i - 1), i0 = i < 0 ? 0 : in_end(i - 1);
+        if (i < 0) {
+            for (int t = 0; t < PRO_W; ++t) { q.push(t, 1); k.w_iss[t] = i; }
+            for (int t = 0; t < PRO_IN; ++t) { q.push(t, 0); k.in_iss[t] = i; }
+            for (int t = PRO_W; t < w_end(i); ++t) { q.push(t, 1); k.w_iss[t] = i; }
+            for (int t = PRO_IN; t < in_end(i); ++t) { q.push(t, 0); k.in_iss[t] = i; }
+        } else {
+            for (int t = w0; t < w_end(i); ++t) { q.push(t, 1); k.w_iss[t] = i; }
+            for (int t = i0; t < in_end(i); ++t) { q.push(t, 0); k.in_iss[t] = i; }
+        }
+        if (i + 1 == RDB_STEPS) break;
+        int tw = tail_w(i), ti = tail_in(i), j = q.n;
+        while (j > landed && (tw > 0 || ti > 0)) {
+            --j;
+            if (q.w[j]) tw -= 1 + TAB.s[q.step[j]].kind; else --ti;
+            if (tw < 0 || ti < 0) { k.ok = false; break; }
+        }
+        if (tw != 0 || ti != 0) k.ok = false;
+        for (; landed < j; ++landed) (q.w[landed] ? k.w_land : k.in_land)[q.step[landed]] = i + 1;
         ++k.bars[2];
-        const int f = in_end(i - 1), e = in_end(i);
-        if (w_pair(i)) { q_step[qn] = i + 1; q_w[qn++] = 1; k.w_iss[i + 1] = i; }
-        else if (w_slab(i)) {
-            if (e - f != 1) k.ok = false;
-            q_step[qn] = f; q_w[qn++] = 1; k.w_iss[f] = i;
-        }
-        for (int t = f; t < e; ++t) { q_step[qn] = t; q_w[qn++] = 0; k.in_iss[t] = i; }
-        tail = tail_w(i) + tail_in(i);
-        if (tail_w(i) && tail_in(i) != e - f) k.ok = false;
-    }
-    if (qn != 2 * RDB_STEPS) k.ok = false;
-    land(qn, RDB_STEPS);
+    }
+    if (q.n != 2 * RDB_STEPS) k.ok = false;
+    for (; landed < q.n; ++landed) (q.w[landed] ? k.w_land : k.in_land)[q.step[landed]] = RDB_STEPS;
     for (int r = 0; r < 2; ++r)
         for (int i = -1; i < RDB_STEPS; ++i) {
-            for (int t = k.rd_lo[r][i + 1]; t <= k.rd_hi[r][i + 1]; ++t) {
+            for (int t = READS.lo[r][i + 1]; t <= READS.hi[r][i + 1]; ++t) {
                 if (k.in_land[t] > i) k.ok = false;
                 for (int u = t + 1; u < RDB_STEPS; ++u) if ((u & 3) == (t & 3) && k.in_iss[u] <= i) k.ok = false;
             }
-            for (int t = k.rd_lo[r][i + 1]; t <= k.wr_hi[r][i + 1]; ++t) {
+            for (int t = READS.lo[r][i + 1]; t <= READS.whi[r][i + 1]; ++t) {
                 if (k.w_land[t] > i) k.ok = false;
-                for (int u = t + 1; u < RDB_STEPS; ++u) if (pos_overlap_w(t, u) && k.w_iss[u] <= i) k.ok = false;
-            }
-        }
+                for (int u = t + 1; u < RDB_STEPS; ++u) if (w_overlap(t, u) && k.w_iss[u] <= i) k.ok = false;
+            }
+        }
+    for (int s = 0; s < RDB_STEPS; ++s) {
+        const int need = TAB.s[s].chunk < 4 ? 0 : ((TAB.s[s].chunk - 4) >> 1) + 1;
+        if (need == 0) continue;
+        int pub = RDB_STEPS;
+        for (int i = 0; i < RDB_STEPS; ++i) if (publish(i) == need) pub = i;
+        if (k.in_iss[s] <= pub) k.ok = false;
+    }
     return k;
 }
 constexpr Walk WALK = walk();
-static_assert(WALK.ok, "a ring position is refilled while it is read, or read before the wait that covers it");
+static_assert(WALK.ok, "a ring position is refilled while it is read, or read before the wait that covers it, or x_j is polled for before it is published");
 static_assert(WALK.bars[0] == RDB_STEPS + 1 && WALK.bars[1] == RDB_STEPS + 1 && WALK.bars[2] == RDB_STEPS + 1, "every role takes the same number of barriers");
 }
 
```
